# chenxing1999/recsys-benchmark

Hardware: AMD Instinct MI355X
Metric: samples/sec fwd+bwd, Criteo-26field DeepFM b=4096; HBM GB/s vs roofline (higher is better)
Workload: dtype f32; 1 GPU; C2 DeepFM Criteo-26field full embedding: F=26, D=16, N=33762577 rows, MLP 400x3+BN+dropout0.5, B=4096/GPU, fwd+bwd, 16 distinct uniform-id batches rotated (fresh ids every step), row-form (COO) table grads, criterion evaluated in the head launch (model(x, labels=y)), next batch known one step ahead (its table rows touched by riders of the weight-gradient launch), tables stored as one packed [N,32]; global_batch=4096, parallelism=single

## Files before the change

recsys-benchmark_amd/csrc/tail.hip:

```cpp
#include <cstdlib>
#include <type_traits>

#include "common.hpp"
#include "tail_gemm.hpp"
#include "tail_masks.hpp"

namespace {
using namespace mi;
using namespace tg;

__device__ __forceinline__ Drop make_drop(const uint8_t *bits, float p, int ld) {
  Drop d;
  d.bits = p > 0.f ? bits : nullptr;
  d.inv_keep = p > 0.f ? 1.f / (1.f - p) : 1.f;
  d.ld = ld;
  return d;
}

__global__ __launch_bounds__(kBlock) void k_tail_dropmask(MaskJob j, const int64_t *seed, float4 *__restrict__ zero4, int64_t nzero4) {
  mask_blocks(j, seed, zero4, nzero4, blockIdx.x, gridDim.x);
}

constexpr int kTilePitch = BNT + 4;
__device__ __forceinline__ void acc_to_lds(const floatx4 (&acc)[NSUB], float *T, int wave, int lane) {
  if (wave < 4) {
    const int r = lane & 15, g = lane >> 4;
    float *row = T + (wave * 16 + r) * kTilePitch + 4 * g;
#pragma unroll
    for (int s = 0; s < NSUB; ++s) st4(row + 16 * s, make_float4(acc[s][0], acc[s][1], acc[s][2], acc[s][3]));
  }
}

__device__ __forceinline__ float sum16(float v) {
  v += __shfl_xor(v, 1); v += __shfl_xor(v, 2); v += __shfl_xor(v, 4); v += __shfl_xor(v, 8);
  return v;
}

struct ActDesc {
  const float *Z;
  int ld;
  const float *mu, *sc, *be;
  float p;
  const uint8_t *keep;
};
__device__ __forceinline__ LoadAct make_act(const ActDesc &d) {
  LoadAct a;
  a.Z = d.Z; a.ld = d.ld; a.mu = d.mu; a.sc = d.sc; a.be = d.be;
  a.drop = make_drop(d.keep, d.p, d.ld);
  return a;
}
struct DzDesc {
  const float *DY, *Z;
  int ld;
  const float *mu, *al, *bz, *de;
};
__device__ __forceinline__ LoadDz make_dz(const DzDesc &d) {
  LoadDz l;
  l.DY = d.DY; l.Z = d.Z; l.ld = d.ld; l.mu = d.mu; l.al = d.al; l.bz = d.bz; l.de = d.de;
  return l;
}


constexpr int kCstPitch = 1024;
constexpr int kCstFloats = 4 * kCstPitch;

struct BnFwd {
  const float *part, *gamma, *beta, *mean_offset;
  float *running_mean, *running_var;
  int64_t *nbt, *seed_bump;
  float *mu, *sc, *be, *rstd;
  float momentum, eps;
  int nrep;
  const float *shift;
};
template <int NT>
__device__ __forceinline__ void bn_derive_fwd(const BnFwd &b, int M, int N, float *cst, bool writer, int tid) {
  const double inv_m = 1.0 / (double)M;
  const double *P = reinterpret_cast<const double *>(b.part);
  for (int n = tid * 2; n < N; n += NT * 2) {
    double t1x = 0.0, t1y = 0.0, t2x = 0.0, t2y = 0.0;
    for (int r = 0; r < b.nrep; ++r) {
      const double2 a = *reinterpret_cast<const double2 *>(P + (int64_t)(2 * r) * N + n);
      const double2 q = *reinterpret_cast<const double2 *>(P + (int64_t)(2 * r + 1) * N + n);
      t1x += a.x; t1y += a.y; t2x += q.x; t2y += q.y;
    }
    const float2 sh = *reinterpret_cast<const float2 *>(b.shift + n);
    const float2 gm2 = b.gamma ? *reinterpret_cast<const float2 *>(b.gamma + n) : make_float2(1.f, 1.f);
    const float2 bt2 = b.beta ? *reinterpret_cast<const float2 *>(b.beta + n) : make_float2(0.f, 0.f);
    float2 mo2 = make_float2(0.f, 0.f), rm2 = mo2, rv2 = mo2;
    if (writer && b.running_mean) {
      rm2 = *reinterpret_cast<const float2 *>(b.running_mean + n);
      rv2 = *reinterpret_cast<const float2 *>(b.running_var + n);
      if (b.mean_offset) mo2 = *reinterpret_cast<const float2 *>(b.mean_offset + n);
    }
#pragma unroll
    for (int j = 0; j < 2; ++j) {
      const int col = n + j;
      const double s1 = j ? t1y : t1x, s2 = j ? t2y : t2x;
      const double dm = s1 * inv_m;
      const float mean = (float)((double)(j ? sh.y : sh.x) + dm);
      const float m2 = fmaxf((float)(s2 - s1 * dm), 0.f);
      const float var = m2 * (float)inv_m;
      const float rstd = rsqrtf(var + b.eps);
      const float gm = j ? gm2.y : gm2.x, bt = j ? bt2.y : bt2.x;
      cst[col] = mean;
      cst[kCstPitch + col] = gm * rstd;
      cst[2 * kCstPitch + col] = bt;
      if (writer) {
        b.mu[col] = mean;
        b.sc[col] = gm * rstd;
        b.be[col] = bt;
        b.rstd[col] = rstd;
// ... 103 lines not shown
  for (int n = tid * 2; n < N; n += NT * 2) {
    const float *p = b.part + (int64_t)n * 2;
    const float2 r2 = *reinterpret_cast<const float2 *>(b.rstd + n), mu2 = *reinterpret_cast<const float2 *>(b.mu + n);
    const float2 gm2 = b.gamma ? *reinterpret_cast<const float2 *>(b.gamma + n) : make_float2(1.f, 1.f);
    float s10 = 0.f, s20 = 0.f, s11 = 0.f, s21 = 0.f;
    for (int base = 0; base < b.nblk; base += CH) {
      float4 v[CH];
#pragma unroll
      for (int u = 0; u < CH; ++u) v[u] = ld4(p + (int64_t)min(base + u, b.nblk - 1) * N * 2);
#pragma unroll
      for (int u = 0; u < CH; ++u)
        if (base + u < b.nblk) { s10 += v[u].x; s20 += v[u].y; s11 += v[u].z; s21 += v[u].w; }
    }
#pragma unroll
    for (int j = 0; j < 2; ++j) {
      const int col = n + j;
      const float s1 = j ? s11 : s10, s2 = j ? s21 : s20;
      const float r = j ? r2.y : r2.x, gm = j ? gm2.y : gm2.x;
      const float dg = s2 * r;
      const float al = gm * r, bz = b.affine ? 0.f : -gm * r * r * dg * inv_m, de = b.affine ? 0.f : -gm * r * s1 * inv_m;
      cst[col] = j ? mu2.y : mu2.x;
      cst[kCstPitch + col] = al;
      cst[2 * kCstPitch + col] = bz;
      cst[3 * kCstPitch + col] = de;
      if (writer) {
        if (b.dgamma) b.dgamma[col] = dg;
        if (b.dbeta) b.dbeta[col] = s1;
        if (b.affine && b.dbias) b.dbias[col] = al * s1;
        b.al[col] = al; b.bz[col] = bz; b.de[col] = de;
      }
    }
  }
  if (wwriter && b.wpart) {
    for (int n = tid; n <= N; n += NT) {
      float sw = 0.f;
      for (int base = 0; base < b.nwblk; base += CH) {
        float v[CH];
#pragma unroll
        for (int u = 0; u < CH; ++u) v[u] = b.wpart[(int64_t)min(base + u, b.nwblk - 1) * (N + 4) + n];
#pragma unroll
        for (int u = 0; u < CH; ++u)
          if (base + u < b.nwblk) sw += v[u];
      }
      if (n < N) b.dw[n] = sw;
      else {
        if (b.db) b.db[0] = sw;
        if (b.db2) b.db2[0] = sw;
      }
    }
  }
}
__device__ __forceinline__ lds_cfp as_lds(const float *p) { return (lds_cfp)p; }

struct FwdArgs {
  ActDesc x;
  const float *W;
  int ldw;
  float *Z;
  int ldz;
  float *part;
  float *a_out;
  int M, N, K;
  int ncols;
  int ntn;
  BnFwd bn;
  int stat_rep;
  float *stat_shift;
  const float *stat_rm, *stat_off;
  const float *head_w, *head_b, *head_add, *h_mu, *h_sc, *h_be;
  float *head_out;
};

template <bool ACT, bool MERGE, bool DMA = false, int NS = NSUB>
__global__ __launch_bounds__(kThreads) void k_tail_fwd(FwdArgs a) {
  __shared__ __attribute__((aligned(16))) float lds[DMA ? kDmaLdsFloats : kLdsFloats + (MERGE ? kCstFloats : 0)];
  const int mt_total = (a.M + BM - 1) / BM;
  const int tile = xcd_logical(blockIdx.x, mt_total * a.ntn);
  if (tile < 0) return;

  const int mt = tile / a.ntn, nt = tile % a.ntn;
  const int m0 = mt * BM, n0 = nt * a.ncols;
  const int rows_valid = min(BM, a.M - m0), cols_valid = min(a.ncols, a.N - n0);
  const int lane = threadIdx.x & 63, wave = threadIdx.x >> 6;
  floatx4 acc[NSUB];
#pragma unroll
  for (int s = 0; s < NSUB; ++s) acc[s] = floatx4{0.f, 0.f, 0.f, 0.f};

  const LoadAct act = make_act(a.x);
  const LoadPlain xp{a.x.Z, a.x.ld};
  const LoadPlain wp{a.W, a.ldw};
  const KcOperand<NS * 16, LoadPlain> opC{wp, n0, cols_valid, a.K};
  if constexpr (MERGE) {
    const lds_cfp c = as_lds(lds + kLdsFloats);
    const LoadActL actl{a.x.Z, a.x.ld, c, c + kCstPitch, c + 2 * kCstPitch, act.drop};
    float *cst = lds + kLdsFloats;
    const bool writer = tile == 0;
    main_loop<true, true>(acc, lds, 0, a.K, KcOperand<64, Tee<LoadActL>>{Tee<LoadActL>{actl, nt == 0 ? a.a_out : nullptr, a.x.ld}, m0, rows_valid, a.K}, opC,
                          make_pre([&]() { bn_merge_fwd<kThreads - kProd>(a.bn, a.M, a.K, cst, writer, (int)threadIdx.x); }));
  } else if constexpr (DMA && ACT)
    main_loop_dma(acc, lds, 0, a.K, KcOperand<64, Tee<LoadAct>, 128>{Tee<LoadAct>{act, nt == 0 ? a.a_out : nullptr, a.x.ld}, m0, rows_valid, a.K},
                  a.W, a.ldw, n0, cols_valid);
  else if constexpr (DMA)
    main_loop_dma(acc, lds, 0, a.K, KcOperand<64, LoadPlain, 128>{xp, m0, rows_valid, a.K}, a.W, a.ldw, n0, cols_valid);
  else if constexpr (ACT)
    main_loop<true, true, NS>(acc, lds, 0, a.K, KcOperand<64, Tee<LoadAct>>{Tee<LoadAct>{act, nt == 0 ? a.a_out : nullptr, a.x.ld}, m0, rows_valid, a.K}, opC);
  else main_loop<true, true, NS>(acc, lds, 0, a.K, KcOperand<64, LoadPlain>{xp, m0, rows_valid, a.K}, opC);

  float *T = lds;
  acc_to_lds(acc, T, wave, lane);
  __syncthreads();
  const int t = threadIdx.x;
  if (a.head_w) {
    const int row = t >> 3, part = t & 7;
    float sum = 0.f;
    if (row < rows_valid) {
#pragma unroll
      for (int j = 0; j < 4; ++j) {
        const int c = (part + 8 * j) * 4;
        if (c < cols_valid) {
          const float4 z = ld4(T + row * kTilePitch + c);
          const float4 u = ld4(a.h_mu + n0 + c), sc = ld4(a.h_sc + n0 + c), be = ld4(a.h_be + n0 + c), w = ld4(a.head_w + n0 + c);
          sum += fmaxf(fmaf(z.x - u.x, sc.x, be.x), 0.f) * w.x + fmaxf(fmaf(z.y - u.y, sc.y, be.y), 0.f) * w.y +
                 fmaxf(fmaf(z.z - u.z, sc.z, be.z), 0.f) * w.z + fmaxf(fmaf(z.w - u.w, sc.w, be.w), 0.f) * w.w;
        }
      }
    }
    sum += __shfl_xor(sum, 1);
    sum += __shfl_xor(sum, 2);
    sum += __shfl_xor(sum, 4);
    if (part == 0 && row < rows_valid) {
      if (nt == 0) sum += (a.head_b ? a.head_b[0] : 0.f) + (a.head_add ? a.head_add[m0 + row] : 0.f);
      atomicAdd(a.head_out + m0 + row, sum);
    }
    return;
  }
#pragma unroll
  for (int k = 0; k < 4; ++k) {
    const int i = t + k * kThreads, row = i / 28, c = (i % 28) * 4;
    if (i < 64 * 28 && row < rows_valid && c < cols_valid)
      st4(a.Z + (int64_t)(m0 + row) * a.ldz + n0 + c, ld4(T + row * kTilePitch + c));
  }
  if (!a.part) return;
  float stat_s = 0.f;
  if (a.stat_rep > 0 && t < cols_valid) {
    if (a.stat_rm) stat_s = a.stat_rm[n0 + t];
    if (a.stat_off) stat_s -= a.stat_off[n0 + t];
  }
  float *ws = lds + 64 * kTilePitch;
  {
    const int col = t & 127, rg = t >> 7;
    const int cnt = max(0, min(16, a.M - (m0 + rg * 16)));
    if (col < cols_valid && cnt > 0) {
      const float *p = T + rg * 16 * kTilePitch + col;
      const float shift = p[0];
      float s1 = 0.f, s2 = 0.f;
      for (int rr = 1; rr < cnt; ++rr) {
        const float d = p[rr * kTilePitch] - shift;
        s1 += d;
        s2 += d * d;
      }
      float *o = ws + (rg * BNT + col) * 3;
      o[0] = shift; o[1] = s1; o[2] = s2;
    }
  }
  __syncthreads();
  if (t < cols_valid) {
    float n_a = 0.f, mean_a = 0.f, m2_a = 0.f;
#pragma unroll
    for (int w = 0; w < 4; ++w) {
      const int cw = max(0, min(16, a.M - (m0 + w * 16)));
      if (cw == 0) continue;
      const float *o = ws + (w * BNT + t) * 3;
      const float n_b = (float)cw, mean_b = o[0] + o[1] / n_b, m2_b = o[2] - o[1] * o[1] / n_b;
      const float n = n_a + n_b, delta = mean_b - mean_a;
      mean_a += delta * (n_b / n);
      m2_a += m2_b + delta * delta * (n_a * n_b / n);
      n_a = n;
    }
    if (a.stat_rep > 0) {
      const double d = (double)mean_a - (double)stat_s;
      double *o = reinterpret_cast<double *>(a.part) + (int64_t)((mt % a.stat_rep) * 2) * a.N + n0 + t;
      atomicAdd(o, (double)n_a * d);
      atomicAdd(o + a.N, (double)n_a * d * d + (double)m2_a);
      if (mt == 0) a.stat_shift[n0 + t] = stat_s;
    } else {
      float *o = a.part + ((int64_t)mt * a.N + n0 + t) * 2;
      o[0] = mean_a;
      o[1] = m2_a;
    }
  }
}

// ... 395 lines not shown
  if (n < N) {
    const int per = (nblk + kFinGroups - 1) / kFinGroups, t0 = grp * per, t1 = min(nblk, t0 + per);
    for (int base = t0; base < t1; base += 16) {
      float2 v[16];
#pragma unroll
      for (int u = 0; u < 16; ++u) v[u] = *reinterpret_cast<const float2 *>(part + ((int64_t)min(base + u, t1 - 1) * N + n) * 2);
#pragma unroll
      for (int u = 0; u < 16; ++u)
        if (base + u < t1) { s1 += v[u].x; s2 += v[u].y; }
    }
  }
  if (wpart && n <= N) {
    const int per = (nwblk + kFinGroups - 1) / kFinGroups, t0 = grp * per, t1 = min(nwblk, t0 + per);
    for (int base = t0; base < t1; base += 16) {
      float v[16];
#pragma unroll
      for (int u = 0; u < 16; ++u) v[u] = wpart[(int64_t)min(base + u, t1 - 1) * (N + 4) + n];
#pragma unroll
      for (int u = 0; u < 16; ++u)
        if (base + u < t1) sw += v[u];
    }
  }
  sh[grp][cl][0] = s1; sh[grp][cl][1] = s2; sh[grp][cl][2] = sw;
  __syncthreads();
  if (grp != 0 || n > N) return;
  s1 = 0.f; s2 = 0.f; sw = 0.f;
#pragma unroll
  for (int q = 0; q < kFinGroups; ++q) { s1 += sh[q][cl][0]; s2 += sh[q][cl][1]; sw += sh[q][cl][2]; }
  if (wpart) {
    if (n < N) dw[n] = sw;
    else {
      if (db) db[0] = sw;
      if (db2) db2[0] = sw;
    }
  }
  if (n >= N) return;
  const float dg = s2 * r;
  if (dgamma) dgamma[n] = dg;
  if (dbeta) dbeta[n] = s1;
  const float inv_m = 1.f / (float)M;
  al[n] = gm * r;
  bz[n] = affine ? 0.f : -gm * r * r * dg * inv_m;
  de[n] = affine ? 0.f : -gm * r * s1 * inv_m;
  if (affine && dbias) dbias[n] = gm * r * s1;
}

__global__ __launch_bounds__(kBlock) void k_tail_affine_consts(AffineJob j) {
  affine_consts_blocks(j, (int)blockIdx.x, (int)gridDim.x);
}

struct DgradArgs {
  DzDesc dz;
  const float *W;
  int ldw;
  ActDesc prev;
  float *OUT;
  int ldo;
  float *part;
  int part_rep;
  float *dz_out;
  int M, N, K;
  int ncols, ntn;
  BnBwd bn;
  const float *fm_emb;
  const float *fm_sum;
  const float *fm_gy;
  float *fm_g1;
  int fm_D;
  const int64_t *fm_slot;
  int fm_pitch;
};

template <bool DZ, bool MID, bool MERGE, bool FM = false>
__global__ __launch_bounds__(kThreads) void k_tail_dgrad(DgradArgs a) {
  __shared__ __attribute__((aligned(16))) float lds[kLdsFloats + (MERGE ? kCstFloats : 0)];
  const int mt_total = (a.M + BM - 1) / BM;
  const int tile = xcd_logical(blockIdx.x, mt_total * a.ntn);
  if (tile < 0) return;

  const int mt = tile / a.ntn, nt = tile % a.ntn;
  const int m0 = mt * BM, k0 = nt * a.ncols;
  const int rows_valid = min(BM, a.M - m0), cols_valid = min(a.ncols, a.K - k0);
  const int lane = threadIdx.x & 63, wave = threadIdx.x >> 6;
  floatx4 acc[NSUB];
#pragma unroll
  for (int s = 0; s < NSUB; ++s) acc[s] = floatx4{0.f, 0.f, 0.f, 0.f};

  const LoadDz dzl = make_dz(a.dz);
  const LoadPlain dyp{a.dz.DY, a.dz.ld};
  const LoadPlain wp{a.W, a.ldw};
  const OtOperand<BNT, LoadPlain> opC{wp, k0, cols_valid, a.N};
  if constexpr (MERGE) {
    const lds_cfp c = as_lds(lds + kLdsFloats);
    const LoadDzL dzm{a.dz.DY, a.dz.Z, a.dz.ld, c, c + kCstPitch, c + 2 * kCstPitch, c + 3 * kCstPitch};
    float *cst = lds + kLdsFloats;
    const bool writer = tile == 0, wwriter = tile == min(1, mt_total * a.ntn - 1);
    main_loop<true, true>(acc, lds, 0, a.N, KcOperand<64, Tee<LoadDzL>>{Tee<LoadDzL>{dzm, nt == 0 ? a.dz_out : nullptr, a.dz.ld}, m0, rows_valid, a.N}, opC,
                          make_pre([&]() { bn_merge_bwd<kThreads - kProd>(a.bn, a.M, a.N, cst, writer, wwriter, (int)threadIdx.x); }));
  } else if constexpr (DZ)
    main_loop<true, true>(acc, lds, 0, a.N, KcOperand<64, Tee<LoadDz>>{Tee<LoadDz>{dzl, nt == 0 ? a.dz_out : nullptr, a.dz.ld}, m0, rows_valid, a.N}, opC);
  else main_loop<true, true>(acc, lds, 0, a.N, KcOperand<64, LoadPlain>{dyp, m0, rows_valid, a.N}, opC);

  float *T = lds;
  acc_to_lds(acc, T, wave, lane);
  __syncthreads();
  const int t = threadIdx.x;
  if constexpr (FM) {
    static_assert(!MID, "the FM epilogue belongs to the product whose output is the tail's input gradient");
    float4 e[4], sm[4], da[4];
    float gy[4];
    int64_t sl[4] = {0, 0, 0, 0};
    bool ok[4];
#pragma unroll
    for (int k = 0; k < 4; ++k) {
      const int i = t + k * kThreads, row = i / 28, c = (i % 28) * 4;
      ok[k] = i < 64 * 28 && row < rows_valid && c < cols_valid;
      const int m = m0 + (ok[k] ? row : 0), kc = k0 + (ok[k] ? c : 0);
      e[k] = ld4(a.fm_emb + (int64_t)m * a.K + kc);
      sm[k] = ld4(a.fm_sum + (int64_t)m * a.fm_D + kc % a.fm_D);
      gy[k] = a.fm_gy[m];
      da[k] = ld4(T + (ok[k] ? row : 0) * kTilePitch + (ok[k] ? c : 0));
      if (a.fm_slot) sl[k] = a.fm_slot[(int64_t)m * (a.K / a.fm_D) + kc / a.fm_D];
    }
#pragma unroll
    for (int k = 0; k < 4; ++k) {
      const int i = t + k * kThreads, row = i / 28, c = (i % 28) * 4;
      if (ok[k]) {
        float4 o;
        o.x = da[k].x + gy[k] * (sm[k].x - e[k].x);
        o.y = da[k].y + gy[k] * (sm[k].y - e[k].y);
        o.z = da[k].z + gy[k] * (sm[k].z - e[k].z);
        o.w = da[k].w + gy[k] * (sm[k].w - e[k].w);
        if (a.fm_slot) {
          float *dst = a.OUT + sl[k] * a.fm_pitch;
          const int d = (k0 + c) % a.fm_D;
          st4(dst + d, o);
          if (d == 0) dst[a.fm_D] = gy[k];
        } else {
          st4(a.OUT + (int64_t)(m0 + row) * a.ldo + k0 + c, o);
        }
      }
    }
    if (a.fm_g1 && nt == 0) {
      const int F = a.K / a.fm_D;
      for (int i = t; i < rows_valid * F; i += kThreads) a.fm_g1[(int64_t)m0 * F + i] = a.fm_gy[m0 + i / F];
    }
  } else if constexpr (!MID) {
#pragma unroll
    for (int k = 0; k < 4; ++k) {
      const int i = t + k * kThreads, row = i / 28, c = (i % 28) * 4;
      if (i < 64 * 28 && row < rows_valid && c < cols_valid)
        st4(a.OUT + (int64_t)(m0 + row) * a.ldo + k0 + c, ld4(T + row * kTilePitch + c));
    }
  } else {
    const Drop drop = make_drop(a.prev.keep, a.prev.p, a.prev.ld);
    const int cg = t % 28, rl = t / 28, c = cg * 4, kc = k0 + c;
    const bool cv = rl < 18 && c < cols_valid;
    float4 s_dy = zero4(), s_dyz = zero4();
    if (cv) {
      const float4 u = ld4(a.prev.mu + kc), sc = ld4(a.prev.sc + kc), be = ld4(a.prev.be + kc);
      float4 z[4], da[4];
      uint32_t kb[4];
#pragma unroll
      for (int k = 0; k < 4; ++k) {
        const int row = rl + 18 * k;
        const int rc = row < rows_valid ? row : rows_valid - 1;
        z[k] = ld4(a.prev.Z + (int64_t)(m0 + rc) * a.prev.ld + kc);
        kb[k] = drop.fetch(m0 + rc, kc);
        da[k] = ld4(T + (row < 64 ? row : 63) * kTilePitch + c);
      }
#pragma unroll
      for (int k = 0; k < 4; ++k) {
        const int row = rl + 18 * k;
        if (row < rows_valid) {
          const float4 kk = drop.scale4(kb[k], kc);
          const float4 zc = make_float4(z[k].x - u.x, z[k].y - u.y, z[k].z - u.z, z[k].w - u.w);
          float4 dy;
          dy.x = fmaf(zc.x, sc.x, be.x) > 0.f ? da[k].x * kk.x : 0.f;
          dy.y = fmaf(zc.y, sc.y, be.y) > 0.f ? da[k].y * kk.y : 0.f;
          dy.z = fmaf(zc.z, sc.z, be.z) > 0.f ? da[k].z * kk.z : 0.f;
          dy.w = fmaf(zc.w, sc.w, be.w) > 0.f ? da[k].w * kk.w : 0.f;
          st4(a.OUT + (int64_t)(m0 + row) * a.ldo + kc, dy);
          s_dy.x += dy.x; s_dy.y += dy.y; s_dy.z += dy.z; s_dy.w += dy.w;
          s_dyz.x += dy.x * zc.x; s_dyz.y += dy.y * zc.y; s_dyz.z += dy.z * zc.z; s_dyz.w += dy.w * zc.w;
        }
      }
    }
// ... 523 lines not shown
```

recsys-benchmark_amd/csrc/tail_gemm.hpp:

```cpp
#pragma once
#include <hip/hip_runtime.h>
#include <stdint.h>

namespace tg {

typedef float floatx4 __attribute__((ext_vector_type(4)));

constexpr int kThreads = 512;
constexpr int kProd = 256;
constexpr int kWaveLanes = 64;
constexpr int BM = 64;
constexpr int BK = 32;
constexpr int NSUB = 7;
constexpr int BNT = NSUB * 16;
constexpr int SR_OC = 68;
constexpr int SC_OC = 116;

__device__ __forceinline__ float4 vld4(const float *p) { return *reinterpret_cast<const float4 *>(p); }
typedef const __attribute__((address_space(3))) float *lds_cfp;
__device__ __forceinline__ float4 vld4(lds_cfp p) {
  const floatx4 v = *reinterpret_cast<const __attribute__((address_space(3))) floatx4 *>(p);
  return make_float4(v[0], v[1], v[2], v[3]);
}
__device__ __forceinline__ void vst4(float *p, float4 v) { *reinterpret_cast<float4 *>(p) = v; }
// ... 413 lines not shown
  L ld;
  int row0, rows_valid, red_end;
  __device__ __forceinline__ int row_of(int i) const {
    const int trow = (ptid() >> 3) + i * (NP / 8);
    return trow < rows_valid ? trow : rows_valid - 1;
  }
  __device__ __forceinline__ KcPrep<ROWS, L, NP> prep() const {
    KcPrep<ROWS, L, NP> p;
    p.cc = (ptid() & 7) << 2;
#pragma unroll
    for (int i = 0; i < NV; ++i) {
      const int trow = (ptid() >> 3) + i * (NP / 8);
      p.lofs[i] = trow < ROWS ? kc_off(trow, ptid() & 7) : -1;
      p.tc[i] = ld.tconst(row_of(i), p.cc);
    }
    return p;
  }
  __device__ __forceinline__ KcStage<ROWS, L, NP> fetch(const KcPrep<ROWS, L, NP> &p, int red0) const {
    KcStage<ROWS, L, NP> st;
    const auto ub = ld.ubase(row0, red0);
    if constexpr (!L::kLateConsts) st.k = ld.consts_u(ub, p.cc);
#pragma unroll
    for (int i = 0; i < NV; ++i) st.raw[i] = ld.fetch_u(ub, p.tc[i]);
    return st;
  }
  __device__ __forceinline__ void finish(float *T, const KcStage<ROWS, L, NP> &st, const KcPrep<ROWS, L, NP> &p, int red0) const {
    const auto ub = ld.ubase(row0, red0);
    typename L::Consts k = st.k;
    if constexpr (L::kLateConsts) k = ld.consts_u(ub, p.cc);
#pragma unroll
    for (int i = 0; i < NV; ++i)
      if ((ROWS * 8) % NP == 0 || i + 1 < NV || p.lofs[i] >= 0) vst4(T + p.lofs[i], ld.finish_u(st.raw[i], k, ub, p.tc[i]));
  }
  __device__ __forceinline__ KcStage<ROWS, L, NP> fetch_any(const KcPrep<ROWS, L, NP> &p, int red0) const {
    KcStage<ROWS, L, NP> st;
    const auto ub = ld.ubase(row0, red0);
    const int rem = red_end - red0;
    const bool dead = p.cc >= rem;
    if constexpr (!L::kLateConsts) st.k = ld.consts_u(ub, dead ? rem - 4 : p.cc);
#pragma unroll
    for (int i = 0; i < NV; ++i) {
      const typename L::TC re = ld.tconst(row_of(i), rem - 4);
      st.raw[i] = ld.fetch_u(ub, dead ? re : p.tc[i]);
    }
    return st;
  }
  __device__ __forceinline__ void finish_any(float *T, const KcStage<ROWS, L, NP> &st, const KcPrep<ROWS, L, NP> &p, int red0) const {
    const auto ub = ld.ubase(row0, red0);
    const int rem = red_end - red0;
    const bool dead = p.cc >= rem;
    typename L::Consts k = st.k;
    if constexpr (L::kLateConsts) k = ld.consts_u(ub, dead ? rem - 4 : p.cc);
#pragma unroll
    for (int i = 0; i < NV; ++i) {
      if ((ROWS * 8) % NP == 0 || i + 1 < NV || p.lofs[i] >= 0) {
        const typename L::TC re = ld.tconst(row_of(i), rem - 4);
        float4 v = ld.finish_u(st.raw[i], k, ub, dead ? re : p.tc[i]);
        if (dead) v = zero4();
        vst4(T + p.lofs[i], v);
      }
    }
  }
};
template <int WIDTH, int S, class L>
struct OcOperand {
  L ld;
  int out0, out_valid, red_end;
  __device__ __forceinline__ OcMap<WIDTH, L> prep() const { return oc_prepare<WIDTH, S>(ld, out0, out_valid); }
  __device__ __forceinline__ OcStage<WIDTH, L> fetch(const OcMap<WIDTH, L> &m, int red0) const { return oc_fetch<WIDTH>(ld, m, red0, red_end); }
  __device__ __forceinline__ void finish(float *T, const OcStage<WIDTH, L> &st, const OcMap<WIDTH, L> &m, int red0) const {
    oc_finish<WIDTH>(T, ld, st, m, red0, red_end);
  }
  __device__ __forceinline__ OcStage<WIDTH, L> fetch_any(const OcMap<WIDTH, L> &m, int red0) const { return fetch(m, red0); }
  __device__ __forceinline__ void finish_any(float *T, const OcStage<WIDTH, L> &st, const OcMap<WIDTH, L> &m, int red0) const { finish(T, st, m, red0); }
};

__device__ __forceinline__ float4 kc_frag(const float *T, int row, int h, int g) { return vld4(T + kc_off(row, 4 * h + g)); }
template <int S>
__device__ __forceinline__ float4 oc_frag(const float *T, int col, int h, int g) {
  const float *p = T + (16 * h + 4 * g) * S + col;
  return make_float4(p[0], p[S], p[2 * S], p[3 * S]);
}

template <int NS>
struct Frags {
  float4 b, a[NS];
};
template <bool R_KC, bool C_KC, int NS>
__device__ __forceinline__ void read_frags(Frags<NS> &f, const float *Rt, const float *Ct, int wave, int lane, int h) {
  const int r = lane & 15, g = lane >> 4;
  f.b = R_KC ? kc_frag(Rt, wave * 16 + r, h, g) : oc_frag<SR_OC>(Rt, wave * 16 + r, h, g);
#pragma unroll
  for (int s = 0; s < NS; ++s) f.a[s] = C_KC ? kc_frag(Ct, s * 16 + r, h, g) : oc_frag<SC_OC>(Ct, s * 16 + r, h, g);
}
template <int NS>
__device__ __forceinline__ void mma_half(floatx4 (&acc)[NSUB], const Frags<NS> &f) {
#pragma unroll
  for (int s = 0; s < NS; ++s) acc[s] = __builtin_amdgcn_mfma_f32_16x16x4f32(f.a[s].x, f.b.x, acc[s], 0, 0, 0);
#pragma unroll
  for (int s = 0; s < NS; ++s) acc[s] = __builtin_amdgcn_mfma_f32_16x16x4f32(f.a[s].y, f.b.y, acc[s], 0, 0, 0);
#pragma unroll
  for (int s = 0; s < NS; ++s) acc[s] = __builtin_amdgcn_mfma_f32_16x16x4f32(f.a[s].z, f.b.z, acc[s], 0, 0, 0);
#pragma unroll
  for (int s = 0; s < NS; ++s) acc[s] = __builtin_amdgcn_mfma_f32_16x16x4f32(f.a[s].w, f.b.w, acc[s], 0, 0, 0);
}

constexpr int kStageFloats = 64 * BK + BNT * BK > 32 * SR_OC + 32 * SC_OC ? 64 * BK + BNT * BK : 32 * SR_OC + 32 * SC_OC;
constexpr int kRing = 4;
constexpr int kLdsFloats = kRing * kStageFloats;
constexpr int kROffKC = 0, kCOffKC = 64 * BK;
constexpr int kROffOC = 0, kCOffOC = 32 * SR_OC;

__device__ __forceinline__ void producer_barrier() {
  __builtin_amdgcn_s_waitcnt(0xC07F);
  __builtin_amdgcn_s_barrier();
}
__device__ __forceinline__ void consumer_barrier() { __builtin_amdgcn_s_barrier(); }

struct NoPre {
  static constexpr bool kActive = false;
  __device__ __forceinline__ void operator()() const {}
};
template <class F>
struct Pre {
  static constexpr bool kActive = true;
  F f;
  __device__ __forceinline__ void operator()() const { f(); }
};
template <class F>
__device__ __forceinline__ Pre<F> make_pre(F f) { return Pre<F>{f}; }

template <bool R_KC, bool C_KC, int NS = NSUB, class OR, class OC, class PRE = NoPre>
__device__ __forceinline__ void main_loop(floatx4 (&acc)[NSUB], float *lds, int red_begin, int red_end, const OR &opR,
                                          const OC &opC, const PRE &pre = PRE{}) {
  const int lane = threadIdx.x & 63, wave = threadIdx.x >> 6;
  constexpr int rOff = R_KC ? kROffKC : kROffOC, cOff = C_KC ? kCOffKC : kCOffOC;
  const int nst = (red_end - red_begin + BK - 1) / BK;
  if (nst <= 0) return;
  const bool partial = (red_end - red_begin) % BK != 0;
  const bool lone = partial && nst == 1;
  auto at = [&](int i) {
    const int ii = i < nst ? i : nst - 1;
    return red_begin + (partial ? (ii == 0 ? nst - 1 : ii - 1) : ii) * BK;
  };
  auto slot = [&](int i) { return lds + (i % kRing) * kStageFloats; };
  if (lone) {
    if (wave >= 4) {
      const auto pR = opR.prep();
      const auto pC = opC.prep();
      const auto r0 = opR.fetch_any(pR, red_begin);
      const auto c0 = opC.fetch_any(pC, red_begin);
      if constexpr (PRE::kActive) producer_barrier();
      opR.finish_any(slot(0) + rOff, r0, pR, red_begin);
      opC.finish_any(slot(0) + cOff, c0, pC, red_begin);
      producer_barrier();
    } else {
      if constexpr (PRE::kActive) {
        pre();
        producer_barrier();
      }
      consumer_barrier();
      Frags<NS> f0, f1;
      read_frags<R_KC, C_KC, NS>(f0, slot(0) + rOff, slot(0) + cOff, wave, lane, 0);
      read_frags<R_KC, C_KC, NS>(f1, slot(0) + rOff, slot(0) + cOff, wave, lane, 1);
      mma_half(acc, f0);
      mma_half(acc, f1);
    }
    __syncthreads();
    return;
  }
  if (wave >= 4) {
    const auto pR = opR.prep();
    const auto pC = opC.prep();
    auto fetchR = [&](int red0) { return opR.fetch(pR, red0); };
    auto fetchC = [&](int red0) { return opC.fetch(pC, red0); };
    auto finishR = [&](float *T, const auto &st, int red0) { opR.finish(T, st, pR, red0); };
    auto finishC = [&](float *T, const auto &st, int red0) { opC.finish(T, st, pC, red0); };
    auto r0 = opR.fetch_any(pR, at(0));
    auto c0 = opC.fetch_any(pC, at(0));
    auto r1 = fetchR(at(1));
    auto c1 = fetchC(at(1));
    auto r2 = fetchR(at(2));
    auto c2 = fetchC(at(2));
    if constexpr (PRE::kActive) producer_barrier();
    opR.finish_any(slot(0) + rOff, r0, pR, at(0));
    opC.finish_any(slot(0) + cOff, c0, pC, at(0));
    r0 = fetchR(at(3));
    c0 = fetchC(at(3));
    if (nst > 1) {
      finishR(slot(1) + rOff, r1, at(1));
      finishC(slot(1) + cOff, c1, at(1));
    }
    r1 = fetchR(at(4));
    c1 = fetchC(at(4));
    if (nst > 2) {
      finishR(slot(2) + rOff, r2, at(2));
      finishC(slot(2) + cOff, c2, at(2));
    }
    r2 = fetchR(at(5));
    c2 = fetchC(at(5));
    producer_barrier();
    for (int i = 0; i < nst; i += 3) {
      if (i + 3 < nst) {
        finishR(slot(i + 3) + rOff, r0, at(i + 3));
        finishC(slot(i + 3) + cOff, c0, at(i + 3));
      }
      r0 = fetchR(at(i + 6));
      c0 = fetchC(at(i + 6));
      producer_barrier();
      if (i + 1 >= nst) break;
      if (i + 4 < nst) {
        finishR(slot(i + 4) + rOff, r1, at(i + 4));
        finishC(slot(i + 4) + cOff, c1, at(i + 4));
      }
      r1 = fetchR(at(i + 7));
      c1 = fetchC(at(i + 7));
      producer_barrier();
      if (i + 2 >= nst) break;
      if (i + 5 < nst) {
        finishR(slot(i + 5) + rOff, r2, at(i + 5));
        finishC(slot(i + 5) + cOff, c2, at(i + 5));
      }
      r2 = fetchR(at(i + 8));
      c2 = fetchC(at(i + 8));
      producer_barrier();
    }
  } else {
    Frags<NS> f0, f1;
    if constexpr (PRE::kActive) {
      pre();
      producer_barrier();
    }
    __builtin_amdgcn_s_setprio(3);
    consumer_barrier();
    read_frags<R_KC, C_KC, NS>(f0, slot(0) + rOff, slot(0) + cOff, wave, lane, 0);
    for (int i = 0; i < nst; ++i) {
      const float *T = slot(i), *Tn = slot(i + 1);
      read_frags<R_KC, C_KC, NS>(f1, T + rOff, T + cOff, wave, lane, 1);
      __builtin_amdgcn_sched_barrier(0);
      mma_half(acc, f0);
      __builtin_amdgcn_sched_barrier(0);
      if (i + 1 < nst) read_frags<R_KC, C_KC, NS>(f0, Tn + rOff, Tn + cOff, wave, lane, 0);
      __builtin_amdgcn_sched_barrier(0);
      mma_half(acc, f1);
      __builtin_amdgcn_sched_barrier(0);
      consumer_barrier();
    }
  }
  __syncthreads();
}


constexpr int kRSlots = 4, kCSlots = 6;
constexpr int kRSlotFloats = 64 * BK, kCSlotFloats = BNT * BK;
constexpr int kDmaLdsFloats = kRSlots * kRSlotFloats + kCSlots * kCSlotFloats;
constexpr int kDmaPerSlice = BNT * 8 / kWaveLanes;
static_assert(kDmaPerSlice == 14, "two loader waves take 7 each");

__device__ __forceinline__ void dma_c_slice(const float *W, int ldw, int n0, int cols_valid, int red0, int red_end, float *slot,
                                            int lw , int lane) {
  const int cpos = lane & 7;
#pragma unroll
  for (int jj = 0; jj < kDmaPerSlice / 2; ++jj) {
    const int j = 2 * jj + lw;
    const int row = 8 * j + (lane >> 3);
    const int chunk = cpos ^ ((row >> 1) & 7);
    const int rc = row < cols_valid ? row : cols_valid - 1;
    int red = red0 + 4 * chunk;
    red = red < red_end ? red : red_end - 4;
    const float *src = W + (int64_t)(n0 + rc) * ldw + red;
    __builtin_amdgcn_global_load_lds((const __attribute__((address_space(1))) void *)src,
                                     (__attribute__((address_space(3))) void *)(slot + j * 256), 16, 0, 0);
  }
}

template <int NS = NSUB, class OR>
__device__ __forceinline__ void main_loop_dma(floatx4 (&acc)[NSUB], float *lds, int red_begin, int red_end, const OR &opR,
                                              const float *W, int ldw, int n0, int cols_valid) {
  const int lane = threadIdx.x & 63, wave = threadIdx.x >> 6;
  const int nst = (red_end - red_begin + BK - 1) / BK;
  if (nst <= 0) return;
  const bool partial = (red_end - red_begin) % BK != 0;
  auto at = [&](int i) {
    const int ii = i < nst ? i : nst - 1;
    return red_begin + (partial ? (ii == 0 ? nst - 1 : ii - 1) : ii) * BK;
  };
  auto rslot = [&](int i) { return lds + (i % kRSlots) * kRSlotFloats; };
  auto cslot = [&](int i) { return lds + kRSlots * kRSlotFloats + (i % kCSlots) * kCSlotFloats; };
  if (wave >= 6) {
    const int lw = wave - 6;
    for (int s = 0; s < 5; ++s)
      if (s < nst) dma_c_slice(W, ldw, n0, cols_valid, at(s), red_end, cslot(s), lw, lane);
    if (nst > 4) asm volatile("s_waitcnt vmcnt(21)" ::: "memory");
    else asm volatile("s_waitcnt vmcnt(0)" ::: "memory");
    __builtin_amdgcn_s_barrier();
    for (int i = 0; i < nst; ++i) {
      if (i + 5 < nst) dma_c_slice(W, ldw, n0, cols_valid, at(i + 5), red_end, cslot(i + 5), lw, lane);
      const int newer = min(nst - 1, i + 5) - min(nst - 1, i + 2);
      if (newer >= 3) asm volatile("s_waitcnt vmcnt(21)" ::: "memory");
      else if (newer == 2) asm volatile("s_waitcnt vmcnt(14)" ::: "memory");
      else if (newer == 1) asm volatile("s_waitcnt vmcnt(7)" ::: "memory");
      else asm volatile("s_waitcnt vmcnt(0)" ::: "memory");
      __builtin_amdgcn_s_barrier();
    }
  } else if (wave >= 4) {
    const auto pR = opR.prep();
    auto fetchR = [&](int red0) { return opR.fetch(pR, red0); };
    auto finishR = [&](float *T, const auto &st, int red0) { opR.finish(T, st, pR, red0); };
    auto r0 = opR.fetch_any(pR, at(0));
    auto r1 = fetchR(at(1));
    auto r2 = fetchR(at(2));
    opR.finish_any(rslot(0), r0, pR, at(0));
    r0 = fetchR(at(3));
    if (nst > 1) finishR(rslot(1), r1, at(1));
    r1 = fetchR(at(4));
    if (nst > 2) finishR(rslot(2), r2, at(2));
    r2 = fetchR(at(5));
    producer_barrier();
    for (int i = 0; i < nst; i += 3) {
      if (i + 3 < nst) finishR(rslot(i + 3), r0, at(i + 3));
      r0 = fetchR(at(i + 6));
      producer_barrier();
      if (i + 1 >= nst) break;
      if (i + 4 < nst) finishR(rslot(i + 4), r1, at(i + 4));
      r1 = fetchR(at(i + 7));
      producer_barrier();
      if (i + 2 >= nst) break;
      if (i + 5 < nst) finishR(rslot(i + 5), r2, at(i + 5));
      r2 = fetchR(at(i + 8));
      producer_barrier();
    }
  } else {
// ... 27 lines not shown
```

Baseline: 18.10 million samples/s.

## Cover ragged column tails with 4x4 MFMA groups and skip dead reduction halves

When a tile's valid columns end four past a multiple of 16 (e.g. 400 = 25*16), the consumer waves now compute only the full 16-column subtiles and cover the remaining four columns with a 4x4x1 MFMA group accumulator. Shuffles reduce that accumulator in the epilogue before storing to LDS. It also skips the second half-step of the partial first stage when the remainder fits in half a BK. The aim is to cut wasted MFMA work on padded columns and reduction slack, at the cost of extra template instantiations, more register pressure from the extra accumulator, and cross-lane reductions in the epilogue.

```diff
diff --git a/recsys-benchmark_amd/csrc/tail.hip b/recsys-benchmark_amd/csrc/tail.hip
--- a/recsys-benchmark_amd/csrc/tail.hip
+++ b/recsys-benchmark_amd/csrc/tail.hip
@@ -22,12 +22,27 @@
 }
 
 constexpr int kTilePitch = BNT + 4;
-__device__ __forceinline__ void acc_to_lds(const floatx4 (&acc)[NSUB], float *T, int wave, int lane) {
+__device__ __forceinline__ void acc_to_lds(const floatx4 (&acc)[NSUB], const floatx4 (&accg)[NGRP], Cover cv, float *T, int wave,
+                                           int lane) {
   if (wave < 4) {
     const int r = lane & 15, g = lane >> 4;
-    float *row = T + (wave * 16 + r) * kTilePitch + 4 * g;
-#pragma unroll
-    for (int s = 0; s < NSUB; ++s) st4(row + 16 * s, make_float4(acc[s][0], acc[s][1], acc[s][2], acc[s][3]));
+    float *row = T + (wave * 16 + r) * kTilePitch;
+#pragma unroll
+    for (int s = 0; s < NSUB; ++s)
+      if (s < cv.nfull) st4(row + 16 * s + 4 * g, make_float4(acc[s][0], acc[s][1], acc[s][2], acc[s][3]));
+#pragma unroll
+    for (int q = 0; q < NGRP; ++q) {
+      if (q < cv.rem) {
+        float v[4];
+#pragma unroll
+        for (int c = 0; c < 4; ++c) {
+          v[c] = accg[q][c];
+          v[c] += __shfl_xor(v[c], 16);
+          v[c] += __shfl_xor(v[c], 32);
+        }
+        if (g == q) st4(row + 16 * cv.nfull + 4 * q, make_float4(v[0], v[1], v[2], v[3]));
+      }
+    }
   }
 }
 
@@ -297,9 +312,12 @@
   const int m0 = mt * BM, n0 = nt * a.ncols;
   const int rows_valid = min(BM, a.M - m0), cols_valid = min(a.ncols, a.N - n0);
   const int lane = threadIdx.x & 63, wave = threadIdx.x >> 6;
-  floatx4 acc[NSUB];
+  floatx4 acc[NSUB], accg[NGRP];
 #pragma unroll
   for (int s = 0; s < NSUB; ++s) acc[s] = floatx4{0.f, 0.f, 0.f, 0.f};
+#pragma unroll
+  for (int q = 0; q < NGRP; ++q) accg[q] = floatx4{0.f, 0.f, 0.f, 0.f};
+  Cover cv{NSUB, 0};
 
   const LoadAct act = make_act(a.x);
   const LoadPlain xp{a.x.Z, a.x.ld};
@@ -310,19 +328,23 @@
     const LoadActL actl{a.x.Z, a.x.ld, c, c + kCstPitch, c + 2 * kCstPitch, act.drop};
     float *cst = lds + kLdsFloats;
     const bool writer = tile == 0;
-    main_loop<true, true>(acc, lds, 0, a.K, KcOperand<64, Tee<LoadActL>>{Tee<LoadActL>{actl, nt == 0 ? a.a_out : nullptr, a.x.ld}, m0, rows_valid, a.K}, opC,
-                          make_pre([&]() { bn_merge_fwd<kThreads - kProd>(a.bn, a.M, a.K, cst, writer, (int)threadIdx.x); }));
+    cv = main_loop_cover(acc, accg, cols_valid, lds, 0, a.K, KcOperand<64, Tee<LoadActL>>{Tee<LoadActL>{actl, nt == 0 ? a.a_out : nullptr, a.x.ld}, m0, rows_valid, a.K}, opC,
+                    make_pre([&]() { bn_merge_fwd<kThreads - kProd>(a.bn, a.M, a.K, cst, writer, (int)threadIdx.x); }));
   } else if constexpr (DMA && ACT)
     main_loop_dma(acc, lds, 0, a.K, KcOperand<64, Tee<LoadAct>, 128>{Tee<LoadAct>{act, nt == 0 ? a.a_out : nullptr, a.x.ld}, m0, rows_valid, a.K},
                   a.W, a.ldw, n0, cols_valid);
   else if constexpr (DMA)
     main_loop_dma(acc, lds, 0, a.K, KcOperand<64, LoadPlain, 128>{xp, m0, rows_valid, a.K}, a.W, a.ldw, n0, cols_valid);
-  else if constexpr (ACT)
-    main_loop<true, true, NS>(acc, lds, 0, a.K, KcOperand<64, Tee<LoadAct>>{Tee<LoadAct>{act, nt == 0 ? a.a_out : nullptr, a.x.ld}, m0, rows_valid, a.K}, opC);
-  else main_loop<true, true, NS>(acc, lds, 0, a.K, KcOperand<64, LoadPlain>{xp, m0, rows_valid, a.K}, opC);
+  else if constexpr (NS != NSUB) {
+    if constexpr (ACT)
+      main_loop<true, true, NS>(acc, lds, 0, a.K, KcOperand<64, Tee<LoadAct>>{Tee<LoadAct>{act, nt == 0 ? a.a_out : nullptr, a.x.ld}, m0, rows_valid, a.K}, opC);
+    else main_loop<true, true, NS>(acc, lds, 0, a.K, KcOperand<64, LoadPlain>{xp, m0, rows_valid, a.K}, opC);
+  } else if constexpr (ACT)
+    cv = main_loop_cover(acc, accg, cols_valid, lds, 0, a.K, KcOperand<64, Tee<LoadAct>>{Tee<LoadAct>{act, nt == 0 ? a.a_out : nullptr, a.x.ld}, m0, rows_valid, a.K}, opC);
+  else cv = main_loop_cover(acc, accg, cols_valid, lds, 0, a.K, KcOperand<64, LoadPlain>{xp, m0, rows_valid, a.K}, opC);
 
   float *T = lds;
-  acc_to_lds(acc, T, wave, lane);
+  acc_to_lds(acc, accg, cv, T, wave, lane);
   __syncthreads();
   const int t = threadIdx.x;
   if (a.head_w) {
@@ -884,9 +906,12 @@
   const int m0 = mt * BM, k0 = nt * a.ncols;
   const int rows_valid = min(BM, a.M - m0), cols_valid = min(a.ncols, a.K - k0);
   const int lane = threadIdx.x & 63, wave = threadIdx.x >> 6;
-  floatx4 acc[NSUB];
+  floatx4 acc[NSUB], accg[NGRP];
 #pragma unroll
   for (int s = 0; s < NSUB; ++s) acc[s] = floatx4{0.f, 0.f, 0.f, 0.f};
+#pragma unroll
+  for (int q = 0; q < NGRP; ++q) accg[q] = floatx4{0.f, 0.f, 0.f, 0.f};
+  Cover cv{NSUB, 0};
 
   const LoadDz dzl = make_dz(a.dz);
   const LoadPlain dyp{a.dz.DY, a.dz.ld};
@@ -897,14 +922,14 @@
     const LoadDzL dzm{a.dz.DY, a.dz.Z, a.dz.ld, c, c + kCstPitch, c + 2 * kCstPitch, c + 3 * kCstPitch};
     float *cst = lds + kLdsFloats;
     const bool writer = tile == 0, wwriter = tile == min(1, mt_total * a.ntn - 1);
-    main_loop<true, true>(acc, lds, 0, a.N, KcOperand<64, Tee<LoadDzL>>{Tee<LoadDzL>{dzm, nt == 0 ? a.dz_out : nullptr, a.dz.ld}, m0, rows_valid, a.N}, opC,
-                          make_pre([&]() { bn_merge_bwd<kThreads - kProd>(a.bn, a.M, a.N, cst, writer, wwriter, (int)threadIdx.x); }));
+    cv = main_loop_cover(acc, accg, cols_valid, lds, 0, a.N, KcOperand<64, Tee<LoadDzL>>{Tee<LoadDzL>{dzm, nt == 0 ? a.dz_out : nullptr, a.dz.ld}, m0, rows_valid, a.N}, opC,
+                    make_pre([&]() { bn_merge_bwd<kThreads - kProd>(a.bn, a.M, a.N, cst, writer, wwriter, (int)threadIdx.x); }));
   } else if constexpr (DZ)
-    main_loop<true, true>(acc, lds, 0, a.N, KcOperand<64, Tee<LoadDz>>{Tee<LoadDz>{dzl, nt == 0 ? a.dz_out : nullptr, a.dz.ld}, m0, rows_valid, a.N}, opC);
-  else main_loop<true, true>(acc, lds, 0, a.N, KcOperand<64, LoadPlain>{dyp, m0, rows_valid, a.N}, opC);
+    cv = main_loop_cover(acc, accg, cols_valid, lds, 0, a.N, KcOperand<64, Tee<LoadDz>>{Tee<LoadDz>{dzl, nt == 0 ? a.dz_out : nullptr, a.dz.ld}, m0, rows_valid, a.N}, opC);
+  else cv = main_loop_cover(acc, accg, cols_valid, lds, 0, a.N, KcOperand<64, LoadPlain>{dyp, m0, rows_valid, a.N}, opC);
 
   float *T = lds;
-  acc_to_lds(acc, T, wave, lane);
+  acc_to_lds(acc, accg, cv, T, wave, lane);
   __syncthreads();
   const int t = threadIdx.x;
   if constexpr (FM) {
diff --git a/recsys-benchmark_amd/csrc/tail_gemm.hpp b/recsys-benchmark_amd/csrc/tail_gemm.hpp
--- a/recsys-benchmark_amd/csrc/tail_gemm.hpp
+++ b/recsys-benchmark_amd/csrc/tail_gemm.hpp
@@ -519,16 +519,44 @@
   return make_float4(p[0], p[S], p[2 * S], p[3 * S]);
 }
 
-template <int NS>
+constexpr int NGRP = 1;
+template <int NF, int NG = 0>
 struct Frags {
-  float4 b, a[NS];
-};
-template <bool R_KC, bool C_KC, int NS>
-__device__ __forceinline__ void read_frags(Frags<NS> &f, const float *Rt, const float *Ct, int wave, int lane, int h) {
+  float4 b, a[NF > 0 ? NF : 1], q[NG > 0 ? NG : 1];
+};
+template <bool R_KC, bool C_KC, int NF, int NG = 0>
+__device__ __forceinline__ void read_frags(Frags<NF, NG> &f, const float *Rt, const float *Ct, int wave, int lane, int h) {
+  static_assert(NG == 0 || C_KC, "four-column groups read KC tiles");
   const int r = lane & 15, g = lane >> 4;
   f.b = R_KC ? kc_frag(Rt, wave * 16 + r, h, g) : oc_frag<SR_OC>(Rt, wave * 16 + r, h, g);
 #pragma unroll
-  for (int s = 0; s < NS; ++s) f.a[s] = C_KC ? kc_frag(Ct, s * 16 + r, h, g) : oc_frag<SC_OC>(Ct, s * 16 + r, h, g);
+  for (int s = 0; s < NF; ++s) f.a[s] = C_KC ? kc_frag(Ct, s * 16 + r, h, g) : oc_frag<SC_OC>(Ct, s * 16 + r, h, g);
+#pragma unroll
+  for (int q = 0; q < NG; ++q) f.q[q] = kc_frag(Ct, NF * 16 + 4 * q + (lane & 3), h, g);
+}
+template <int J>
+__device__ __forceinline__ float comp(const float4 &v) {
+  if constexpr (J == 0) return v.x;
+  else if constexpr (J == 1) return v.y;
+  else if constexpr (J == 2) return v.z;
+  else return v.w;
+}
+template <int J, int NF, int NG>
+__device__ __forceinline__ void mma_step(floatx4 (&acc)[NSUB], floatx4 (&accg)[NGRP], const Frags<NF, NG> &f) {
+#pragma unroll
+  for (int s = 0; s < NF; ++s) acc[s] = __builtin_amdgcn_mfma_f32_16x16x4f32(comp<J>(f.a[s]), comp<J>(f.b), acc[s], 0, 0, 0);
+  if constexpr (NG > 0) {
+#pragma unroll
+    for (int q = 0; q < NG; ++q) accg[q] = __builtin_amdgcn_mfma_f32_4x4x1f32(comp<J>(f.q[q]), comp<J>(f.b), accg[q], 0, 0, 0);
+    __builtin_amdgcn_sched_barrier(0);
+  }
+}
+template <int NF, int NG>
+__device__ __forceinline__ void mma_half(floatx4 (&acc)[NSUB], floatx4 (&accg)[NGRP], const Frags<NF, NG> &f) {
+  mma_step<0>(acc, accg, f);
+  mma_step<1>(acc, accg, f);
+  mma_step<2>(acc, accg, f);
+  mma_step<3>(acc, accg, f);
 }
 template <int NS>
 __device__ __forceinline__ void mma_half(floatx4 (&acc)[NSUB], const Frags<NS> &f) {
@@ -540,6 +568,12 @@
   for (int s = 0; s < NS; ++s) acc[s] = __builtin_amdgcn_mfma_f32_16x16x4f32(f.a[s].z, f.b.z, acc[s], 0, 0, 0);
 #pragma unroll
   for (int s = 0; s < NS; ++s) acc[s] = __builtin_amdgcn_mfma_f32_16x16x4f32(f.a[s].w, f.b.w, acc[s], 0, 0, 0);
+}
+struct Cover {
+  int nfull, rem;
+};
+__device__ __forceinline__ Cover cover_of(int cols_valid, int red_len) {
+  return (cols_valid & 15) == 4 && red_len >= BK ? Cover{cols_valid >> 4, 1} : Cover{NSUB, 0};
 }
 
 constexpr int kStageFloats = 64 * BK + BNT * BK > 32 * SR_OC + 32 * SC_OC ? 64 * BK + BNT * BK : 32 * SR_OC + 32 * SC_OC;
@@ -567,15 +601,55 @@
 template <class F>
 __device__ __forceinline__ Pre<F> make_pre(F f) { return Pre<F>{f}; }
 
-template <bool R_KC, bool C_KC, int NS = NSUB, class OR, class OC, class PRE = NoPre>
-__device__ __forceinline__ void main_loop(floatx4 (&acc)[NSUB], float *lds, int red_begin, int red_end, const OR &opR,
-                                          const OC &opC, const PRE &pre = PRE{}) {
+template <bool R_KC, bool C_KC, int NF, int NG>
+__device__ __forceinline__ void consume(floatx4 (&acc)[NSUB], floatx4 (&accg)[NGRP], float *lds, int nst, bool dead_half, int wave,
+                                        int lane) {
+  constexpr int rOff = R_KC ? kROffKC : kROffOC, cOff = C_KC ? kCOffKC : kCOffOC;
+  auto slot = [&](int i) { return lds + (i % kRing) * kStageFloats; };
+  Frags<NF, NG> f0, f1;
+  read_frags<R_KC, C_KC, NF, NG>(f0, slot(0) + rOff, slot(0) + cOff, wave, lane, 0);
+  int i = 0;
+  if (dead_half) {
+    __builtin_amdgcn_sched_barrier(0);
+    mma_half(acc, accg, f0);
+    __builtin_amdgcn_sched_barrier(0);
+    if (1 < nst) read_frags<R_KC, C_KC, NF, NG>(f0, slot(1) + rOff, slot(1) + cOff, wave, lane, 0);
+    __builtin_amdgcn_sched_barrier(0);
+    consumer_barrier();
+    i = 1;
+  }
+  for (; i < nst; ++i) {
+    const float *T = slot(i), *Tn = slot(i + 1);
+    read_frags<R_KC, C_KC, NF, NG>(f1, T + rOff, T + cOff, wave, lane, 1);
+    __builtin_amdgcn_sched_barrier(0);
+    mma_half(acc, accg, f0);
+    __builtin_amdgcn_sched_barrier(0);
+    if (i + 1 < nst) read_frags<R_KC, C_KC, NF, NG>(f0, Tn + rOff, Tn + cOff, wave, lane, 0);
+    __builtin_amdgcn_sched_barrier(0);
+    mma_half(acc, accg, f1);
+    __builtin_amdgcn_sched_barrier(0);
+    consumer_barrier();
+  }
+}
+template <int NF>
+__device__ __forceinline__ void consume_cover(floatx4 (&acc)[NSUB], floatx4 (&accg)[NGRP], float *lds, int nst, bool dead_half,
+                                              int wave, int lane, int nfull) {
+  if constexpr (NF < NSUB) {
+    if (nfull == NF) consume<true, true, NF, 1>(acc, accg, lds, nst, dead_half, wave, lane);
+    else consume_cover<NF + 1>(acc, accg, lds, nst, dead_half, wave, lane, nfull);
+  }
+}
+
+template <bool R_KC, bool C_KC, int NS, bool COVER, class OR, class OC, class PRE>
+__device__ __forceinline__ void main_loop_impl(floatx4 (&acc)[NSUB], floatx4 (&accg)[NGRP], Cover cv, float *lds, int red_begin,
+                                               int red_end, const OR &opR, const OC &opC, const PRE &pre) {
   const int lane = threadIdx.x & 63, wave = threadIdx.x >> 6;
   constexpr int rOff = R_KC ? kROffKC : kROffOC, cOff = C_KC ? kCOffKC : kCOffOC;
   const int nst = (red_end - red_begin + BK - 1) / BK;
   if (nst <= 0) return;
   const bool partial = (red_end - red_begin) % BK != 0;
   const bool lone = partial && nst == 1;
+  const bool dead_half = partial && (red_end - red_begin) % BK <= BK / 2;
   auto at = [&](int i) {
     const int ii = i < nst ? i : nst - 1;
     return red_begin + (partial ? (ii == 0 ? nst - 1 : ii - 1) : ii) * BK;
@@ -599,9 +673,11 @@
       consumer_barrier();
       Frags<NS> f0, f1;
       read_frags<R_KC, C_KC, NS>(f0, slot(0) + rOff, slot(0) + cOff, wave, lane, 0);
-      read_frags<R_KC, C_KC, NS>(f1, slot(0) + rOff, slot(0) + cOff, wave, lane, 1);
       mma_half(acc, f0);
-      mma_half(acc, f1);
+      if (!dead_half) {
+        read_frags<R_KC, C_KC, NS>(f1, slot(0) + rOff, slot(0) + cOff, wave, lane, 1);
+        mma_half(acc, f1);
+      }
     }
     __syncthreads();
     return;
@@ -663,28 +739,30 @@
       producer_barrier();
     }
   } else {
-    Frags<NS> f0, f1;
     if constexpr (PRE::kActive) {
       pre();
       producer_barrier();
     }
     __builtin_amdgcn_s_setprio(3);
     consumer_barrier();
-    read_frags<R_KC, C_KC, NS>(f0, slot(0) + rOff, slot(0) + cOff, wave, lane, 0);
-    for (int i = 0; i < nst; ++i) {
-      const float *T = slot(i), *Tn = slot(i + 1);
-      read_frags<R_KC, C_KC, NS>(f1, T + rOff, T + cOff, wave, lane, 1);
-      __builtin_amdgcn_sched_barrier(0);
-      mma_half(acc, f0);
-      __builtin_amdgcn_sched_barrier(0);
-      if (i + 1 < nst) read_frags<R_KC, C_KC, NS>(f0, Tn + rOff, Tn + cOff, wave, lane, 0);
-      __builtin_amdgcn_sched_barrier(0);
-      mma_half(acc, f1);
-      __builtin_amdgcn_sched_barrier(0);
-      consumer_barrier();
-    }
+    if (COVER && cv.rem != 0) {
+      if constexpr (COVER) consume_cover<0>(acc, accg, lds, nst, dead_half, wave, lane, cv.nfull);
+    } else consume<R_KC, C_KC, NS, 0>(acc, accg, lds, nst, dead_half, wave, lane);
   }
   __syncthreads();
+}
+template <bool R_KC, bool C_KC, int NS = NSUB, class OR, class OC, class PRE = NoPre>
+__device__ __forceinline__ void main_loop(floatx4 (&acc)[NSUB], float *lds, int red_begin, int red_end, const OR &opR,
+                                          const OC &opC, const PRE &pre = PRE{}) {
+  floatx4 none[NGRP];
+  main_loop_impl<R_KC, C_KC, NS, false>(acc, none, Cover{NS, 0}, lds, red_begin, red_end, opR, opC, pre);
+}
+template <class OR, class OC, class PRE = NoPre>
+__device__ __forceinline__ Cover main_loop_cover(floatx4 (&acc)[NSUB], floatx4 (&accg)[NGRP], int cols_valid, float *lds, int red_begin,
+                                                 int red_end, const OR &opR, const OC &opC, const PRE &pre = PRE{}) {
+  const Cover cv = cover_of(cols_valid, red_end - red_begin);
+  main_loop_impl<true, true, NSUB, true>(acc, accg, cv, lds, red_begin, red_end, opR, opC, pre);
+  return cv;
 }
 
 
```

Measured after the change: 18.48 million samples/s, median of 6. +2.1%, better.
